# snt-arg/visual_sgraphs

Measured on NVIDIA B200. Metric: orb_extraction_frames_per_s_640x480_1000f, higher is better.
Workload: dtype u8

## Files before the change

visual_sgraphs_b200/csrc/resize_tma.cu:

```cuda
#include <cuda.h>
#include <cuda_runtime.h>

#include <algorithm>
#include <cstdint>
#include <cstdlib>
#include <vector>

#include "tma_util.cuh"
#include "vsg_internal.cuh"

namespace vsg {

constexpr int kRtW = 128, kRtH = 32;
constexpr int kRtBoxW = 192, kRtBoxH = 48;
constexpr int kRtWarps = 8;
constexpr int kRtThreads = 32 * (kRtWarps + 1);
constexpr int kRtHPitch = kRtW + 4;
constexpr int kRtWin = kRtBoxW * kRtBoxH;
constexpr int kRtSmem = 2 * kRtWin + kRtBoxH * kRtHPitch * 4 + 128;

struct RtTileInfo {
    int x0, y0, frame, xs, ys, nrows, ylast, pad;
    short4 yt[kRtH];
};

__global__ void __launch_bounds__(kRtThreads, 4) resize_tma_kernel(const __grid_constant__ CUtensorMap src_map, uint8_t *__restrict__ dst,
                                                                   int dst_pitch, int64_t dst_stride, int dw, int dh, int tiles_x,
                                                                   int tiles_y, int total_tiles, int per_cta,
                                                                   const short4 *__restrict__ xtab, const short4 *__restrict__ ytab) {
    extern __shared__ uint8_t rt_smem_raw[];
    uint8_t *win = reinterpret_cast<uint8_t *>(((uintptr_t)rt_smem_raw + 127) & ~(uintptr_t)127);
    uint32_t *hp = reinterpret_cast<uint32_t *>(win + 2 * kRtWin);
    __shared__ uint64_t full[2], empty[2];
    __shared__ RtTileInfo info[2];
    const int tid = threadIdx.x, lane = tid & 31, warp = tid >> 5;
    const int t_begin = blockIdx.x * per_cta, t_end = min(t_begin + per_cta, total_tiles);
    if (tid == 0) {
        for (int i = 0; i < 2; ++i) { mbar_init(&full[i], 1); mbar_init(&empty[i], kRtWarps); }
        mbar_init_fence();
    }
    __syncthreads();
    const int tiles_per_frame = tiles_x * tiles_y;

    if (warp == kRtWarps) {
        for (int t = t_begin, it = 0; t < t_end; ++t, ++it) {
            const int st = it & 1;
            const int frame = t / tiles_per_frame, rem = t - frame * tiles_per_frame;
            const int tx = rem / tiles_y, ty = rem - tx * tiles_y;
            const int x0 = tx * kRtW, y0 = ty * kRtH, ylast = min(y0 + kRtH, dh) - 1;
            const short4 ytl = __ldg(&ytab[min(y0 + lane, dh - 1)]);
            const int xs = __ldg(&xtab[x0]).x & ~15;
            const int ys = __shfl_sync(0xffffffffu, (int)ytl.x, 0);
            const int nrows = __shfl_sync(0xffffffffu, (int)ytl.y, ylast - y0) - ys + 1;
            mbar_wait(&empty[st], ((it >> 1) & 1) ^ 1);
            info[st].yt[lane] = ytl;
            if (lane == 0) {
                info[st].x0 = x0; info[st].y0 = y0; info[st].frame = frame; info[st].xs = xs; info[st].ys = ys;
                info[st].nrows = nrows; info[st].ylast = ylast;
            }
            __syncwarp();
            if (lane == 0) {
                mbar_expect_tx(&full[st], kRtWin);
                tma_load_3d(win + st * kRtWin, &src_map, xs, ys, frame, &full[st]);
            }
        }
        return;
    }

    int cur_x0 = -1;
    bool col_ok = false;
    uint32_t sel[4], coef[4];
    bool hi[4];
    int base = 0;
    for (int t = t_begin, it = 0; t < t_end; ++t, ++it) {
        const int st = it & 1;
        mbar_wait(&full[st], (it >> 1) & 1);
        const int x0 = info[st].x0, y0 = info[st].y0, frame = info[st].frame, xs = info[st].xs, ys = info[st].ys, nrows = info[st].nrows,
                  ylast = info[st].ylast;
        const int x4 = x0 + 4 * lane;
        if (x0 != cur_x0) {
            cur_x0 = x0;
            col_ok = x4 < dw;
            short4 xt[4];
#pragma unroll
            for (int k = 0; k < 4; ++k) xt[k] = col_ok ? __ldg(&xtab[x4 + k]) : make_short4(0, 0, 0, 0);
            base = xt[0].x & ~3;
#pragma unroll
            for (int k = 0; k < 4; ++k) {
                const int o0 = xt[k].x - base, o1 = xt[k].y - base;
                hi[k] = o1 >= 8;
                const int f = hi[k] ? 4 : 0;
                sel[k] = (uint32_t)(o0 - f) | ((uint32_t)(o1 - f) << 4);
                coef[k] = (uint32_t)(uint16_t)xt[k].z | ((uint32_t)(uint16_t)xt[k].w << 16);
            }
        }
        const uint8_t *wcol = win + st * kRtWin + (col_ok ? base - xs : 0);
        for (int r = warp; r < nrows; r += kRtWarps) {
            const uint32_t *p = reinterpret_cast<const uint32_t *>(wcol + r * kRtBoxW);
            const uint32_t w0 = p[0], w1 = p[1], w2 = p[2];
            uint4 g;
            uint32_t *gp = &g.x;
#pragma unroll
            for (int k = 0; k < 4; ++k) {
                const uint32_t bytes = hi[k] ? __byte_perm(w1, w2, sel[k]) : __byte_perm(w0, w1, sel[k]);
                gp[k] = __dp2a_lo(coef[k], bytes, 0u) >> 4;
            }
            *reinterpret_cast<uint4 *>(hp + r * kRtHPitch + 4 * lane) = g;
        }
        short4 yt[kRtH / kRtWarps];
#pragma unroll
        for (int i = 0; i < kRtH / kRtWarps; ++i) yt[i] = info[st].yt[warp + kRtWarps * i];
        __syncwarp();
        if (lane == 0) mbar_arrive(&empty[st]);
        asm volatile("bar.sync 1, %0;" ::"n"(32 * kRtWarps) : "memory");
        uint8_t *d = dst + (int64_t)frame * dst_stride + x4;
#pragma unroll
        for (int i = 0; i < kRtH / kRtWarps; ++i) {
            const int y = y0 + warp + kRtWarps * i;
            if (y > ylast || !col_ok) continue;
            const uint4 ga = *reinterpret_cast<const uint4 *>(hp + (yt[i].x - ys) * kRtHPitch + 4 * lane);
            const uint4 gb = *reinterpret_cast<const uint4 *>(hp + (yt[i].y - ys) * kRtHPitch + 4 * lane);
            const uint32_t b0 = (uint32_t)yt[i].z << 16, b1 = (uint32_t)yt[i].w << 16;
            const uint32_t v0 = (__umulhi(b0, ga.x) + __umulhi(b1, gb.x) + 2u) >> 2, v1 = (__umulhi(b0, ga.y) + __umulhi(b1, gb.y) + 2u) >> 2;
            const uint32_t v2 = (__umulhi(b0, ga.z) + __umulhi(b1, gb.z) + 2u) >> 2, v3 = (__umulhi(b0, ga.w) + __umulhi(b1, gb.w) + 2u) >> 2;
            *reinterpret_cast<uint32_t *>(d + (int64_t)y * dst_pitch) = v0 | (v1 << 8) | (v2 << 16) | (v3 << 24);
        }
        asm volatile("bar.sync 1, %0;" ::"n"(32 * kRtWarps) : "memory");
    }
}

static int resize_tma_min_frames() {
    const char *e = getenv("VSG_RESIZE_TMA");
    const int v = e ? atoi(e) : 16;
    return v <= 0 ? INT32_MAX : v;
}

bool launch_resize_level_tma(const FrameGeom &g, int level, const uint8_t *src_base, int src_pitch, int64_t src_stride, uint8_t *pyr,
                             int nframes, cudaStream_t s) {
    if (nframes < resize_tma_min_frames()) return false;
    const LevelGeom &L = g.lv[level], &P = g.lv[level - 1];
    if (!L.resize_tma_ok || ((uintptr_t)src_base & 15) || (src_pitch & 15) || (src_stride & 15) || src_pitch < kRtBoxW) return false;
    EncodeTiledFn fn = encode_tiled_fn();
    if (!fn) return false;
    CUtensorMap map;
    const cuuint64_t dims[3] = {(cuuint64_t)src_pitch, (cuuint64_t)P.h, (cuuint64_t)nframes};
    const cuuint64_t strides[2] = {(cuuint64_t)src_pitch, (cuuint64_t)src_stride};
    const cuuint32_t box[3] = {kRtBoxW, kRtBoxH, 1};
    const cuuint32_t estr[3] = {1, 1, 1};
    if (fn(&map, CU_TENSOR_MAP_DATA_TYPE_UINT8, 3, (void *)src_base, dims, strides, box, estr, CU_TENSOR_MAP_INTERLEAVE_NONE,
           CU_TENSOR_MAP_SWIZZLE_NONE, CU_TENSOR_MAP_L2_PROMOTION_L2_128B, CU_TENSOR_MAP_FLOAT_OOB_FILL_NONE) != CUDA_SUCCESS)
        return false;
    if (cudaFuncSetAttribute(resize_tma_kernel, cudaFuncAttributeMaxDynamicSharedMemorySize, kRtSmem) != cudaSuccess) {
        cudaGetLastError();
        return false;
    }
    const int tiles_x = (L.w + kRtW - 1) / kRtW, tiles_y = (L.h + kRtH - 1) / kRtH;
    const int64_t total = (int64_t)tiles_x * tiles_y * nframes;
    if (total > INT32_MAX) return false;
    int dev = 0, sms = 148;
    cudaGetDevice(&dev);
    cudaDeviceGetAttribute(&sms, cudaDevAttrMultiProcessorCount, dev);
    const int ctas = (int)std::min<int64_t>(total, (int64_t)sms * 4);
    const int per_cta = (int)((total + ctas - 1) / ctas);
    resize_tma_kernel<<<(unsigned)((total + per_cta - 1) / per_cta), kRtThreads, kRtSmem, s>>>(
        map, pyr + L.plane_offset, L.pitch, L.plane_stride, L.w, L.h, tiles_x, tiles_y, (int)total, per_cta, L.xtab, L.ytab);
    count_launch();
    return true;
}

bool resize_tma_fits(const std::vector<short4> &xt, const std::vector<short4> &yt, int dw, int dh) {
    for (int x0 = 0; x0 < dw; x0 += kRtW) {
        const int xl = std::min(x0 + kRtW, dw) - 1;
        if ((xt[xl].y & ~3) + 12 - (xt[x0].x & ~15) > kRtBoxW) return false;
    }
    for (int y0 = 0; y0 < dh; y0 += kRtH) {
        const int yl = std::min(y0 + kRtH, dh) - 1;
        if (yt[yl].y - yt[y0].x + 1 > kRtBoxH) return false;
    }
    return true;
}

}
```

visual_sgraphs_b200/csrc/vsg_api.cu:

```cuda
#include <algorithm>
#include <atomic>
#include <cmath>
#include <cstdarg>
#include <cstdio>
#include <cstdlib>
#include <cstring>
#include <vector>

#include "vsg_internal.cuh"

namespace vsg {

static thread_local char g_err[512] = "";
static std::atomic<int64_t> g_launches{0};

void set_error(const char *fmt, ...) {
    va_list ap;
    va_start(ap, fmt);
    vsnprintf(g_err, sizeof(g_err), fmt, ap);
    va_end(ap);
}
bool cuda_ok(cudaError_t e, const char *what) {
    if (e == cudaSuccess) return true;
    set_error("%s: %s", what, cudaGetErrorString(e));
    return false;
}
void count_launch(int n) { g_launches += n; }
static thread_local bool g_pdl_small_batch = true;
constexpr int kPdlMaxFrames = 8;
void pdl_scope(int nframes) { g_pdl_small_batch = nframes <= kPdlMaxFrames; }
bool pdl_enabled() { return g_pdl_small_batch; }

static inline int cv_round(float v) { return (int)lrintf(v); }
static inline int cv_round(double v) { return (int)lrint(v); }
static inline int64_t align_up(int64_t v, int64_t a) { return (v + a - 1) / a * a; }

}

using namespace vsg;

struct vsg_extractor {
    int device = 0;
    int max_batch = 1;
    cudaStream_t stream = nullptr;
    static constexpr int kAuxStreams = 2;
    cudaStream_t aux[kAuxStreams] = {nullptr, nullptr};
    int chunk_frames = 128;
    uint8_t *color_d = nullptr;
    size_t color_bytes = 0;
    uint32_t *rect_xy[2] = {nullptr, nullptr};
    uint16_t *rect_frac[2] = {nullptr, nullptr};
    int rect_w = 0, rect_h = 0;
    cudaEvent_t fork_ev = nullptr;
    vsg_orb_params p{};
    std::vector<float> scale, inv_scale, sigma2, inv_sigma2;
    std::vector<int> quota;

    int cur_w = 0, cur_h = 0;
    FrameGeom g{};
    int max_cw = 0, max_ch = 0, max_nodes = 0;
    int64_t pyr_bytes_per_frame = 0;

    short4 *tabs_d = nullptr;
    PyrTile *pyr_tiles_d = nullptr;
    int pyr_ntiles = 0, pyr_tile_buf = 0;
    size_t pyr_tile_smem = 0;
    uint8_t *pyr = nullptr, *blur = nullptr;
    Cand *cand = nullptr;
    unsigned short *node_of = nullptr;
    int *cand_count = nullptr;
    LevelKp *level_kps = nullptr;
    int *level_kp_count = nullptr;
    int *slot = nullptr;
    uint8_t *out_block_d = nullptr, *out_block_h = nullptr;
    size_t out_block_bytes = 0;
    vsg_keypoint *kps_d = nullptr;
    uint8_t *desc_d = nullptr;
    int *n_d = nullptr, *mono_d = nullptr;
    vsg_keypoint *kps_h = nullptr;
    uint8_t *desc_h = nullptr;
    int *n_h = nullptr, *mono_h = nullptr;

    bool profile = false;
    static constexpr int kEvRing = 32;
    cudaEvent_t ev[kEvRing][VSG_NUM_STAGES + 1] = {};
    bool ev_created = false;
    int ev_head = 0, ev_pending = 0;
    double stage_ms[VSG_NUM_STAGES] = {0, 0, 0, 0, 0};
    int64_t stage_runs = 0;

    void harvest_one() {
        const int slot = (ev_head - ev_pending + 2 * kEvRing) % kEvRing;
        cudaEventSynchronize(ev[slot][VSG_NUM_STAGES]);
        for (int k = 0; k < VSG_NUM_STAGES; ++k) {
            float ms = 0.f;
            cudaEventElapsedTime(&ms, ev[slot][k], ev[slot][k + 1]);
            stage_ms[k] += ms;
        }
        ++stage_runs;
        --ev_pending;
    }

    const uint8_t *lvl0_base = nullptr;
    int lvl0_pitch = 0;
    int64_t lvl0_stride = 0;
    int last_nframes = 0;
    bool results_on_handle = false;

    void free_shape() {
        cudaFree(tabs_d); cudaFree(pyr_tiles_d); cudaFree(pyr); cudaFree(blur); cudaFree(cand); cudaFree(node_of);
        cudaFree(cand_count); cudaFree(level_kps); cudaFree(level_kp_count); cudaFree(slot); cudaFree(out_block_d);
        cudaFree(color_d);
        color_d = nullptr; color_bytes = 0;
        cudaFreeHost(out_block_h);
        out_block_d = out_block_h = nullptr; out_block_bytes = 0;
        tabs_d = nullptr; pyr_tiles_d = nullptr; pyr_ntiles = 0; pyr = blur = nullptr; cand = nullptr; node_of = nullptr;
        cand_count = nullptr; level_kps = nullptr; level_kp_count = nullptr; slot = nullptr; kps_d = nullptr;
        desc_d = nullptr; n_d = mono_d = nullptr; kps_h = nullptr; desc_h = nullptr; n_h = mono_h = nullptr;
        cur_w = cur_h = 0;
    }
};

namespace {

void build_tables(vsg_extractor *ex) {
    const int nl = ex->p.nlevels;
    const double scale_factor = ex->p.scale_factor;
    ex->scale.assign(nl, 1.f);
    ex->sigma2.assign(nl, 1.f);
    for (int i = 1; i < nl; ++i) {
        ex->scale[i] = (float)(ex->scale[i - 1] * scale_factor);
        ex->sigma2[i] = ex->scale[i] * ex->scale[i];
    }
    ex->inv_scale.resize(nl);
    ex->inv_sigma2.resize(nl);
    for (int i = 0; i < nl; ++i) {
        ex->inv_scale[i] = 1.0f / ex->scale[i];
        ex->inv_sigma2[i] = 1.0f / ex->sigma2[i];
    }
    ex->quota.assign(nl, 0);
    const float factor = (float)(1.0f / scale_factor);
    float desired = ex->p.nfeatures * (1 - factor) / (1 - (float)std::pow((double)factor, (double)nl));
    int sum = 0;
    for (int l = 0; l < nl - 1; ++l) {
        ex->quota[l] = cv_round(desired);
        sum += ex->quota[l];
        desired *= factor;
    }
    ex->quota[nl - 1] = std::max(ex->p.nfeatures - sum, 0);
}

void build_resize_tables(int sw, int sh, int dw, int dh, int dw_pad, std::vector<short4> &xt, std::vector<short4> &yt) {
    const double scale_x = 1.0 / ((double)dw / sw), scale_y = 1.0 / ((double)dh / sh);
    xt.resize(dw_pad);
    yt.resize(dh);
    for (int dx = 0; dx < dw_pad; ++dx) {
        const int x = std::min(dx, dw - 1);
        float fx = (float)((x + 0.5) * scale_x - 0.5);
        int sx = (int)std::floor(fx);
        fx -= sx;
        if (sx < 0) { fx = 0; sx = 0; }
        if (sx >= sw - 1) { fx = 0; sx = sw - 1; }
        xt[dx] = make_short4((short)sx, (short)std::min(sx + 1, sw - 1), (short)cv_round((1.f - fx) * 2048.f),
                             (short)cv_round(fx * 2048.f));
    }
    for (int dy = 0; dy < dh; ++dy) {
        float fy = (float)((dy + 0.5) * scale_y - 0.5);
        int sy = (int)std::floor(fy);
        fy -= sy;
        const int sy0 = std::min(std::max(sy, 0), sh - 1), sy1 = std::min(std::max(sy + 1, 0), sh - 1);
        yt[dy] = make_short4((short)sy0, (short)sy1, (short)cv_round((1.f - fy) * 2048.f), (short)cv_round(fy * 2048.f));
    }
}

vsg_status configure_shape(vsg_extractor *ex, int w, int h) {
    if (ex->cur_w == w && ex->cur_h == h) return VSG_OK;
    if (w > kMaxImageDim || h > kMaxImageDim) {
        set_error("image %dx%d too large: at most %d pixels per side", w, h, kMaxImageDim);
        return VSG_ERR_INVALID;
    }
    CK(cudaSetDevice(ex->device));
    int smem_optin = 0;
    size_t octree_static = 0;
    CK(cudaDeviceGetAttribute(&smem_optin, cudaDevAttrMaxSharedMemoryPerBlockOptin, ex->device));
    const vsg_status ost = octree_static_smem_bytes(&octree_static);
    if (ost != VSG_OK) return ost;
    ex->free_shape();
    const int nl = ex->p.nlevels;
    FrameGeom &g = ex->g;
    memset(&g, 0, sizeof(g));
    g.nlevels = nl;
    std::vector<Cell> cells;
    ex->max_cw = ex->max_ch = 7;
    ex->max_nodes = 8;
    int64_t plane_off = 0, cand_off = 0;
    int kp_off = 0;
    std::vector<std::vector<short4>> xts(nl), yts(nl);
    for (int l = 0; l < nl; ++l) {
        LevelGeom &L = g.lv[l];
        L.w = cv_round((float)w * ex->inv_scale[l]);
        L.h = cv_round((float)h * ex->inv_scale[l]);
        const int min_b = kBorderMin, max_bx = L.w - kBorderMin, max_by = L.h - kBorderMin;
        const float width = (float)(max_bx - min_b), height = (float)(max_by - min_b);
        if (width < 35.f || height < 35.f) {
            set_error("image %dx%d too small: level %d is %dx%d (needs >= 67x67 for one 35-px cell)", w, h, l, L.w, L.h);
            return VSG_ERR_INVALID;
        }
        L.pitch = (int)align_up(L.w, 64);
        L.plane_stride = align_up((int64_t)L.pitch * L.h, 256);
        L.plane_offset = plane_off;
        plane_off += L.plane_stride * ex->max_batch;
        L.n_cols = (int)(width / 35.f);
        L.n_rows = (int)(height / 35.f);
        L.w_cell = (int)std::ceil(width / L.n_cols);
        L.h_cell = (int)std::ceil(height / L.n_rows);
        L.cell_begin = (int)cells.size();
        int cand_cap = 0;
        for (int i = 0; i < L.n_rows; ++i) {
            const float ini_y = (float)(min_b + i * L.h_cell);
            float max_y = ini_y + L.h_cell + 6;
            if (ini_y >= max_by - 3) continue;
            if (max_y > max_by) max_y = (float)max_by;
            for (int j = 0; j < L.n_cols; ++j) {
                const float ini_x = (float)(min_b + j * L.w_cell);
                float max_x = ini_x + L.w_cell + 6;
                if (ini_x >= max_bx - 6) continue;
                if (max_x > max_bx) max_x = (float)max_bx;
                Cell c;
                c.level = (short)l;
                c.x0 = (short)ini_x; c.y0 = (short)ini_y;
                c.cw = (short)((int)max_x - (int)ini_x); c.ch = (short)((int)max_y - (int)ini_y);
                c.pad = 0;
                if (c.cw < 7 || c.ch < 7) continue;
                cells.push_back(c);
                ex->max_cw = std::max<int>(ex->max_cw, c.cw);
                ex->max_ch = std::max<int>(ex->max_ch, c.ch);
                cand_cap += ((c.cw - 6 + 1) / 2) * ((c.ch - 6 + 1) / 2);
            }
        }
        L.cell_count = (int)cells.size() - L.cell_begin;
        L.cols_eff = L.rows_eff = 0;
        for (int k = L.cell_begin; k < (int)cells.size(); ++k) {
            const Cell &c = cells[k];
            L.cols_eff = std::max(L.cols_eff, (c.x0 - min_b) / L.w_cell + 1);
            L.rows_eff = std::max(L.rows_eff, (c.y0 - min_b) / L.h_cell + 1);
        }
        if (L.cols_eff * L.rows_eff != L.cell_count) {
            set_error("internal: level %d cell table is not a prefix rectangle", l);
            return VSG_ERR_INVALID;
        }
        L.cols_rcp = (uint32_t)((0x100000000ull + (uint64_t)L.cols_eff - 1) / (uint64_t)std::max(L.cols_eff, 1));
        L.wcell_rcp = L.w_cell > 1 ? (uint32_t)((0x100000000ull + (uint64_t)L.w_cell - 1) / (uint64_t)L.w_cell) : 0xFFFFFFFFu;
        L.hcell_rcp = L.h_cell > 1 ? (uint32_t)((0x100000000ull + (uint64_t)L.h_cell - 1) / (uint64_t)L.h_cell) : 0xFFFFFFFFu;
        L.quota = ex->quota[l];
        L.n_ini = (int)std::round(static_cast<float>(max_bx - min_b) / (max_by - min_b));
        if (L.n_ini < 1) {
            set_error("image %dx%d: aspect ratio below 0.5 is not supported by the reference oct-tree (nIni = 0)", w, h);
            return VSG_ERR_INVALID;
        }
        L.h_x = static_cast<float>(max_bx - min_b) / L.n_ini;
        L.cand_cap = cand_cap + 8;
        L.cand_offset = cand_off;
        cand_off += L.cand_cap;
        L.kp_cap = std::max(L.quota, 4 * L.n_ini) + 4;
        L.kp_offset = kp_off;
        kp_off += L.kp_cap;
        const size_t octree_need = octree_smem_bytes(L.kp_cap + 4) + octree_static;
        if (octree_need > (size_t)smem_optin) {
            set_error("level %d: oct-tree quota %d needs %zu bytes of shared memory per block, the device allows %d", l, L.quota,
                      octree_need, smem_optin);
            return VSG_ERR_INVALID;
        }
        ex->max_nodes = std::max(ex->max_nodes, L.kp_cap + 4);
        L.scale = ex->scale[l];
        L.kp_size = (float)(int)(kPatch * ex->scale[l]);
        L.resize_tma_ok = 0;
        if (l > 0) {
            build_resize_tables(g.lv[l - 1].w, g.lv[l - 1].h, L.w, L.h, (int)align_up(L.w, 4), xts[l], yts[l]);
            L.resize_tma_ok = resize_tma_fits(xts[l], yts[l], L.w, L.h) ? 1 : 0;
        }
    }
    g.ncells = (int)cells.size();
    for (int l = nl; l < kMaxLevels; ++l) g.lv[l].cell_begin = 0x7fffffff;
    g.cand_total = cand_off;
    g.kp_total = kp_off;
    g.out_cap = kp_off;
    ex->pyr_bytes_per_frame = plane_off / ex->max_batch;

    const int B = ex->max_batch;
    size_t ntab = 0;
    for (int l = 1; l < nl; ++l) ntab += xts[l].size() + yts[l].size();
    CK(cudaMalloc(&ex->tabs_d, std::max<size_t>(ntab, 1) * sizeof(short4)));
    size_t toff = 0;
    for (int l = 1; l < nl; ++l) {
        CK(cudaMemcpy(ex->tabs_d + toff, xts[l].data(), xts[l].size() * sizeof(short4), cudaMemcpyHostToDevice));
        g.lv[l].xtab = ex->tabs_d + toff;
        toff += xts[l].size();
        CK(cudaMemcpy(ex->tabs_d + toff, yts[l].data(), yts[l].size() * sizeof(short4), cudaMemcpyHostToDevice));
        g.lv[l].ytab = ex->tabs_d + toff;
        toff += yts[l].size();
    }
    if (nl >= 2) {
        constexpr int ntx = 12, nty = 12;
        std::vector<PyrTile> tiles((size_t)ntx * nty);
        int buf = 0, ntab_max = 0, dim_max = 0;
        for (int ty = 0; ty < nty; ++ty)
            for (int tx = 0; tx < ntx; ++tx) {
                PyrTile &t = tiles[(size_t)ty * ntx + tx];
                int ntab_t = 0;
                for (int l = nl - 1; l >= 0; --l) {
                    const int W = g.lv[l].w, H = g.lv[l].h;
                    PyrTileBox o{(short)(tx * W / ntx), (short)(ty * H / nty), (short)((tx + 1) * W / ntx - 1), (short)((ty + 1) * H / nty - 1)};
                    PyrTileBox r = o;
                    if (l < nl - 1) {
                        const PyrTileBox &u = t.region[l + 1];
                        const short nx0 = xts[l + 1][u.x0].x, nx1 = xts[l + 1][u.x1].y, ny0 = yts[l + 1][u.y0].x, ny1 = yts[l + 1][u.y1].y;
                        if (l == 0) r = PyrTileBox{nx0, ny0, nx1, ny1};
                        else r = PyrTileBox{std::min(o.x0, nx0), std::min(o.y0, ny0), std::max(o.x1, nx1), std::max(o.y1, ny1)};
                    }
                    t.owned[l] = o;
                    t.region[l] = r;
                    t.rcp_w[l] = (uint32_t)((0x100000000ull + (uint64_t)(r.x1 - r.x0)) / (uint64_t)(r.x1 - r.x0 + 1));
                    buf = std::max(buf, (r.x1 - r.x0 + 1) * (r.y1 - r.y0 + 1));
                    if (l > 0) dim_max = std::max(dim_max, std::max(r.x1 - r.x0 + 1, r.y1 - r.y0 + 1));
                    if (l > 0) ntab_t += (r.x1 - r.x0 + 1) + (r.y1 - r.y0 + 1);
                }
                for (int l = nl; l < kMaxLevels; ++l) { t.owned[l] = t.region[l] = PyrTileBox{0, 0, -1, -1}; t.rcp_w[l] = 0; }
                ntab_max = std::max(ntab_max, ntab_t);
            }
        ex->pyr_tile_buf = (int)align_up(buf, 16);
        ex->pyr_tile_smem = 2 * (size_t)ex->pyr_tile_buf + (size_t)ntab_max * sizeof(short4);
        if (ex->pyr_tile_smem <= 160 * 1024 && dim_max <= 256 && buf < 65536 && nl <= kMaxLevels && g.lv[nl - 1].w >= 2 * ntx && g.lv[nl - 1].h >= 2 * nty) {
            CK(cudaMalloc(&ex->pyr_tiles_d, tiles.size() * sizeof(PyrTile)));
            CK(cudaMemcpy(ex->pyr_tiles_d, tiles.data(), tiles.size() * sizeof(PyrTile), cudaMemcpyHostToDevice));
            ex->pyr_ntiles = (int)tiles.size();
        }
    }
    CK(cudaMalloc(&ex->pyr, plane_off + 256));
    CK(cudaMalloc(&ex->blur, plane_off + 256));
    CK(cudaMemset(ex->pyr, 0, plane_off + 256));
    CK(cudaMalloc(&ex->cand, (size_t)g.cand_total * B * sizeof(Cand)));
    CK(cudaMalloc(&ex->node_of, (size_t)g.cand_total * B * sizeof(unsigned short)));
    CK(cudaMalloc(&ex->cand_count, (size_t)B * nl * sizeof(int)));
    CK(cudaMalloc(&ex->level_kps, (size_t)g.kp_total * B * sizeof(LevelKp)));
    CK(cudaMalloc(&ex->level_kp_count, (size_t)B * nl * sizeof(int)));
    CK(cudaMalloc(&ex->slot, (size_t)g.kp_total * B * sizeof(int)));
    {
        auto up = [](size_t v) { return (v + 255) & ~(size_t)255; };
        const size_t off_desc = up((size_t)g.out_cap * B * sizeof(vsg_keypoint));
        const size_t off_n = off_desc + up((size_t)g.out_cap * B * 32);
        const size_t off_mono = off_n + up((size_t)B * sizeof(int));
        ex->out_block_bytes = off_mono + up((size_t)B * sizeof(int));
        CK(cudaMalloc(&ex->out_block_d, ex->out_block_bytes));
        CK(cudaMallocHost(&ex->out_block_h, ex->out_block_bytes));
        ex->kps_d = reinterpret_cast<vsg_keypoint *>(ex->out_block_d);
        ex->desc_d = ex->out_block_d + off_desc;
        ex->n_d = reinterpret_cast<int *>(ex->out_block_d + off_n);
        ex->mono_d = reinterpret_cast<int *>(ex->out_block_d + off_mono);
        ex->kps_h = reinterpret_cast<vsg_keypoint *>(ex->out_block_h);
        ex->desc_h = ex->out_block_h + off_desc;
        ex->n_h = reinterpret_cast<int *>(ex->out_block_h + off_n);
        ex->mono_h = reinterpret_cast<int *>(ex->out_block_h + off_mono);
    }
    ex->cur_w = w;
    ex->cur_h = h;
    return VSG_OK;
}

static int pyr_tile_max_frames() {
    const char *e = getenv("VSG_PYR_TILE");
    return e ? atoi(e) : 4;
}

vsg_status run_pipeline(vsg_extractor *ex, cudaStream_t s, int f0, const uint8_t *lvl0_base, int lvl0_pitch,
                        int64_t lvl0_stride, int nframes, int lap_x0, int lap_x1, vsg_keypoint *kps_dev,
                        uint8_t *desc_dev, int out_cap, int *n_dev, int *mono_dev) {
    FrameGeom g = ex->g;
    for (int l = 0; l < g.nlevels; ++l) {
        g.lv[l].plane_offset += (int64_t)f0 * g.lv[l].plane_stride;
        g.lv[l].cand_offset += (int64_t)f0 * g.cand_total;
    }
    pdl_scope(nframes);
    int *cand_count = ex->cand_count + (size_t)f0 * g.nlevels;
    int *level_kp_count = ex->level_kp_count + (size_t)f0 * g.nlevels;
    LevelKp *level_kps = ex->level_kps + (size_t)f0 * g.kp_total;
    int *slot = ex->slot + (size_t)f0 * g.kp_total;
    CK(cudaMemsetAsync(cand_count, 0, (size_t)nframes * g.nlevels * sizeof(int), s));
    cudaEvent_t *ev = nullptr;
    if (ex->profile && s == ex->stream) {
        if (!ex->ev_created) {
            for (int i = 0; i < vsg_extractor::kEvRing; ++i)
                for (int k = 0; k <= VSG_NUM_STAGES; ++k) CK(cudaEventCreate(&ex->ev[i][k]));
            ex->ev_created = true;
        }
        if (ex->ev_pending == vsg_extractor::kEvRing) ex->harvest_one();
        ev = ex->ev[ex->ev_head];
        ex->ev_head = (ex->ev_head + 1) % vsg_extractor::kEvRing;
        ++ex->ev_pending;
    }
#define STAGE_MARK(k) do { if (ev) CK(cudaEventRecord(ev[k], s)); } while (0)
    STAGE_MARK(0);
    if (ex->pyr_tiles_d && nframes <= pyr_tile_max_frames()) {
        launch_pyramid_tiles(g, ex->pyr_tiles_d, ex->pyr_ntiles, ex->pyr_tile_buf, ex->pyr_tile_smem, lvl0_base, lvl0_pitch, lvl0_stride,
                             ex->pyr, nframes, s);
    } else {
        for (int l = 1; l < g.nlevels; ++l) {
            const LevelGeom &P = g.lv[l - 1];
            if (l == 1) launch_resize_level(g, l, lvl0_base, lvl0_pitch, lvl0_stride, ex->pyr, nframes, s);
            else launch_resize_level(g, l, ex->pyr + P.plane_offset, P.pitch, P.plane_stride, ex->pyr, nframes, s);
        }
    }
    STAGE_MARK(1);
    const BlurTcPlan *blur_tc = plan_blur_tc(g, lvl0_base, lvl0_pitch, lvl0_stride, ex->pyr, ex->blur, nframes);
    const vsg_status fst = launch_fast(g, lvl0_base, lvl0_pitch, lvl0_stride, ex->pyr, blur_tc ? nullptr : ex->blur, ex->cand,
                                       cand_count, ex->p.ini_th_fast, ex->p.min_th_fast, ex->max_cw, ex->max_ch, nframes, s);
    if (fst != VSG_OK) return fst;
    STAGE_MARK(2);
    const vsg_status ost = launch_octree(g, ex->cand, cand_count, ex->node_of, level_kps, level_kp_count, ex->max_nodes, nframes, s);
    if (ost != VSG_OK) return ost;
    STAGE_MARK(3);
    if (blur_tc) launch_blur_tc(blur_tc, ex->blur, s);
    STAGE_MARK(4);
    launch_describe(g, lvl0_base, lvl0_pitch, lvl0_stride, ex->pyr, ex->blur, level_kps, level_kp_count, lap_x0,
                    lap_x1, kps_dev, desc_dev, out_cap, n_dev, mono_dev, slot, nframes, s);
    STAGE_MARK(5);
#undef STAGE_MARK
    CK(cudaGetLastError());
    return VSG_OK;
}

}

namespace vsg {
bool extractor_pyramid(vsg_extractor *ex, PyramidRef *out) {
    if (!ex || ex->cur_w == 0 || ex->last_nframes == 0) return false;
    out->device = ex->device;
    out->nframes = ex->last_nframes;
    out->geom = &ex->g;
    out->lvl0_base = ex->lvl0_base;
    out->lvl0_pitch = ex->lvl0_pitch;
    out->lvl0_stride = ex->lvl0_stride;
    out->pyr = ex->pyr;
    out->scale = ex->scale.data();
    out->inv_scale = ex->inv_scale.data();
    out->stream = ex->stream;
    out->kps_dev = ex->results_on_handle ? ex->kps_d : nullptr;
    out->desc_dev = ex->results_on_handle ? ex->desc_d : nullptr;
    out->n_dev = ex->results_on_handle ? ex->n_d : nullptr;
    out->out_cap = ex->g.out_cap;
    return true;
}
}

extern "C" {

const char *vsg_last_error(void) { return g_err; }

int vsg_device_count(void) {
    int n = 0;
    if (cudaGetDeviceCount(&n) != cudaSuccess) { cudaGetLastError(); return 0; }
    return n;
}

int64_t vsg_launch_count(void) { return g_launches.load(); }

vsg_status vsg_extractor_create(const vsg_orb_params *params, int device, int max_batch, vsg_extractor **out) {
    if (!params || !out || max_batch < 1 || params->nlevels < 1 || params->nlevels > kMaxLevels ||
        params->scale_factor <= 1.0f || params->scale_factor >= 2.0f || params->nfeatures < 0) {
        set_error("vsg_extractor_create: invalid argument");
        return VSG_ERR_INVALID;
    }
    if (vsg_device_count() <= device || device < 0) {
        set_error("vsg_extractor_create: CUDA device %d not available (this library has no CPU fallback)", device);
        return VSG_ERR_CUDA;
    }
    vsg_extractor *ex = new vsg_extractor();
    ex->device = device;
    ex->max_batch = max_batch;
    ex->p = *params;
    build_tables(ex);
    if (!cuda_ok(cudaSetDevice(device), "cudaSetDevice") ||
        !cuda_ok(cudaStreamCreateWithFlags(&ex->stream, cudaStreamNonBlocking), "cudaStreamCreate") ||
        !cuda_ok(cudaStreamCreateWithFlags(&ex->aux[0], cudaStreamNonBlocking), "cudaStreamCreate") ||
        !cuda_ok(cudaStreamCreateWithFlags(&ex->aux[1], cudaStreamNonBlocking), "cudaStreamCreate")) {
        delete ex;
        return VSG_ERR_CUDA;
    }
    if (const char *e = getenv("VSG_CHUNK_FRAMES")) ex->chunk_frames = std::max(1, atoi(e));
    cudaEventCreateWithFlags(&ex->fork_ev, cudaEventDisableTiming);
    *out = ex;
    return VSG_OK;
}

void vsg_extractor_destroy(vsg_extractor *ex) {
    if (!ex) return;
    cudaSetDevice(ex->device);
    if (ex->stream) { cudaStreamSynchronize(ex->stream); cudaStreamDestroy(ex->stream); }
    for (cudaStream_t a : ex->aux)
        if (a) { cudaStreamSynchronize(a); cudaStreamDestroy(a); }
    if (ex->fork_ev) cudaEventDestroy(ex->fork_ev);
    if (ex->ev_created)
        for (int i = 0; i < vsg_extractor::kEvRing; ++i)
            for (int k = 0; k <= VSG_NUM_STAGES; ++k) cudaEventDestroy(ex->ev[i][k]);
    ex->free_shape();
    for (int k = 0; k < 2; ++k) { cudaFree(ex->rect_xy[k]); cudaFree(ex->rect_frac[k]); }
    delete ex;
}

vsg_status vsg_extractor_tables(const vsg_extractor *ex, float *scale, float *inv_scale, float *sigma2,
                                float *inv_sigma2, int32_t *features_per_level) {
    if (!ex) return VSG_ERR_INVALID;
    for (int i = 0; i < ex->p.nlevels; ++i) {
        if (scale) scale[i] = ex->scale[i];
        if (inv_scale) inv_scale[i] = ex->inv_scale[i];
        if (sigma2) sigma2[i] = ex->sigma2[i];
        if (inv_sigma2) inv_sigma2[i] = ex->inv_sigma2[i];
        if (features_per_level) features_per_level[i] = ex->quota[i];
    }
    return VSG_OK;
}

int vsg_extractor_max_keypoints(vsg_extractor *ex, int width, int height) {
    if (!ex) return VSG_ERR_INVALID;
    vsg_status st = configure_shape(ex, width, height);
    if (st != VSG_OK) return st;
    return ex->g.out_cap;
}

static vsg_status extract_batch_host(vsg_extractor *ex, const uint8_t *images, int nframes, int src_w, int src_h, int pitch,
                                     size_t frame_stride, int channels, int r_first, int rect_slots, int lap_x0, int lap_x1,
                                     vsg_keypoint *keypoints_out, uint8_t *descriptors_out, int capacity, int *n_out,
                                     int *mono_index_out) {
    if (!ex) return VSG_ERR_INVALID;
    if (!images || src_w <= 0 || src_h <= 0 || nframes <= 0) return VSG_EMPTY_IMAGE;
    if (nframes > ex->max_batch || pitch < src_w * channels || capacity < 0 || (channels != 1 && channels != 3 && channels != 4)) {
        set_error("vsg_extract_batch: nframes %d > max_batch %d, or bad pitch/capacity/channels", nframes, ex->max_batch);
        return VSG_ERR_INVALID;
    }
    const bool staged = channels != 1 || rect_slots > 0;
    const int width = rect_slots > 0 ? ex->rect_w : src_w, height = rect_slots > 0 ? ex->rect_h : src_h;
    CK(cudaSetDevice(ex->device));
    vsg_status st = configure_shape(ex, width, height);
    if (st != VSG_OK) return st;
    const int cpitch = (src_w * channels + 63) & ~63;
    const size_t cstride = (size_t)cpitch * src_h;
    if (staged && ex->color_bytes < cstride * ex->max_batch) {
        cudaFree(ex->color_d);
        ex->color_d = nullptr; ex->color_bytes = 0;
        CK(cudaMalloc(&ex->color_d, cstride * ex->max_batch));
        ex->color_bytes = cstride * ex->max_batch;
    }
    const FrameGeom &g = ex->g;
    const LevelGeom &L0 = g.lv[0];
    uint8_t *lvl0 = ex->pyr + L0.plane_offset;
    ex->lvl0_base = lvl0; ex->lvl0_pitch = L0.pitch; ex->lvl0_stride = L0.plane_stride; ex->last_nframes = nframes;
    ex->results_on_handle = true;
    auto pinned = [](const void *p) {
        if (!p) return false;
        cudaPointerAttributes a;
        if (cudaPointerGetAttributes(&a, p) != cudaSuccess) { cudaGetLastError(); return false; }
        return a.type == cudaMemoryTypeHost;
    };
    const bool direct = capacity >= g.out_cap && (!keypoints_out || pinned(keypoints_out)) &&
                        (!descriptors_out || pinned(descriptors_out));
    const int min_chunk = std::min(ex->chunk_frames, 64);
    const bool chunked = !ex->profile && nframes >= 2 * min_chunk;
    int chunk = nframes;
    if (chunked) {
        const int nchunks = std::max(2, (nframes + ex->chunk_frames - 1) / ex->chunk_frames);
        chunk = (nframes + nchunks - 1) / nchunks;
    }
    const bool tight = frame_stride == (size_t)pitch * height && (int64_t)L0.pitch * L0.h == L0.plane_stride;
    RectifyMaps maps = {{ex->rect_xy[0], ex->rect_xy[1]}, {ex->rect_frac[0], ex->rect_frac[1]}, rect_slots};
    int nstreams_used = 0;
    if (chunked) {
        CK(cudaEventRecord(ex->fork_ev, ex->stream));
        for (cudaStream_t a : ex->aux) CK(cudaStreamWaitEvent(a, ex->fork_ev, 0));
    }
    for (int f0 = 0, c = 0; f0 < nframes; f0 += chunk, ++c) {
        const int nf = std::min(chunk, nframes - f0);
        cudaStream_t s = (c % 3 == 0) ? ex->stream : ex->aux[c % 3 - 1];
        nstreams_used = std::min(3, c + 1);
// ... 279 lines not shown
```

visual_sgraphs_b200/csrc/vsg_internal.cuh:

```cuda
#pragma once
#include <cuda_runtime.h>
#include <stdint.h>

#include <vector>

#include "../../include/vsg_cuda.h"

namespace vsg {

constexpr int kMaxLevels = 16;
constexpr int kEdge = 19;
constexpr int kBorderMin = 16;
constexpr int kMaxImageDim = 16384;
constexpr int kHalfPatch = 15;
constexpr int kPatch = 31;

struct LevelGeom {
    int w, h;
    int pitch;
    int64_t plane_stride;
    int64_t plane_offset;
    int n_cols, n_rows, w_cell, h_cell;
    int cell_begin, cell_count;
    int cols_eff, rows_eff;
    uint32_t cols_rcp;
    uint32_t wcell_rcp, hcell_rcp;
    int quota;
    int n_ini;
    float h_x;
    int cand_cap;
    int64_t cand_offset;
    int kp_cap;
    int kp_offset;
    float scale;
    float kp_size;
    int resize_tma_ok;
    const short4 *xtab;
    const short4 *ytab;
};

struct FrameGeom {
    int nlevels;
    int ncells;
    int64_t cand_total;
    int kp_total;
    int out_cap;
    LevelGeom lv[kMaxLevels];
};

struct Cell {
    short level;
    short x0, y0;
    short cw, ch;
    short pad;
};

struct __align__(8) Cand {
    unsigned short x, y;
    unsigned short score;
    unsigned short pad;
};

struct __align__(8) LevelKp {
    unsigned short x, y;
    unsigned short score;
    unsigned short pad;
};

}

struct vsg_matcher {
    int device = 0;
    cudaStream_t stream = nullptr;
    void *buf[20] = {};
    size_t cap[20] = {};
    void *hbuf[8] = {};
    size_t hcap[8] = {};
    std::vector<char> scratch[2];
    int sm_count = 148;
};

namespace vsg {

vsg_status matcher_ensure(vsg_matcher *m, int slot, size_t bytes);
vsg_status matcher_ensure_host(vsg_matcher *m, int slot, size_t bytes);
vsg_status launch_knn2_merge_parts(vsg_matcher *m, const int32_t *idx_parts, const int32_t *dist_parts, int nparts, int nq,
                                   int32_t *out_idx, int32_t *out_dist);
bool knn2_tc_supported(int nq, int nt);
vsg_status knn2_tc_device(vsg_matcher *m, const uint8_t *q_dev, int nq, const uint8_t *t_dev, int nt, int offset, int *idx_dev,
                          int *dist_dev);
void launch_window_dists(vsg_matcher *m, const uint8_t *query_dev, int nq, const uint8_t *train_dev,
                         const int *cand_ptr_dev, const int *cand_dev, int *all_dist_dev);

struct PyramidRef {
    int device;
    int nframes;
    const FrameGeom *geom;
    const uint8_t *lvl0_base;
    int lvl0_pitch;
    int64_t lvl0_stride;
    const uint8_t *pyr;
    const float *scale, *inv_scale;
    cudaStream_t stream;
    const vsg_keypoint *kps_dev;
    const uint8_t *desc_dev;
    const int *n_dev;
    int out_cap;
};
bool extractor_pyramid(vsg_extractor *ex, PyramidRef *out);

__device__ __forceinline__ void pdl_launch_dependents() { asm volatile("griddepcontrol.launch_dependents;" ::: "memory"); }
__device__ __forceinline__ void pdl_wait() { asm volatile("griddepcontrol.wait;" ::: "memory"); }
bool pdl_enabled();
void pdl_scope(int nframes);

template <class... KArgs, class... Args>
inline cudaError_t launch_kernel(void (*kernel)(KArgs...), dim3 grid, dim3 block, size_t smem, cudaStream_t s, bool pdl,
                                 Args... args) {
    cudaLaunchConfig_t cfg = {};
    cfg.gridDim = grid;
    cfg.blockDim = block;
    cfg.dynamicSmemBytes = smem;
    cfg.stream = s;
    cudaLaunchAttribute attr[1];
    attr[0].id = cudaLaunchAttributeProgrammaticStreamSerialization;
    attr[0].val.programmaticStreamSerializationAllowed = 1;
    cfg.attrs = attr;
    cfg.numAttrs = (pdl && pdl_enabled()) ? 1 : 0;
    return cudaLaunchKernelEx(&cfg, kernel, KArgs(args)...);
}

void set_error(const char *fmt, ...);
bool cuda_ok(cudaError_t e, const char *what);
#define CK(call)                                          \
    do {                                                  \
        if (!cuda_ok((call), #call)) return VSG_ERR_CUDA; \
    } while (0)
void count_launch(int n = 1);

struct PyrTileBox { short x0, y0, x1, y1; };
struct PyrTile {
    PyrTileBox region[kMaxLevels], owned[kMaxLevels];
    uint32_t rcp_w[kMaxLevels];
};
void launch_pyramid_tiles(const FrameGeom &g, const PyrTile *tiles, int ntiles, int buf_bytes, size_t smem, const uint8_t *lvl0_base,
                          int lvl0_pitch, int64_t lvl0_stride, uint8_t *pyr, int nframes, cudaStream_t s);
bool launch_resize_level_tma(const FrameGeom &g, int level, const uint8_t *src_base, int src_pitch, int64_t src_stride, uint8_t *pyr,
                             int nframes, cudaStream_t s);
bool resize_tma_fits(const std::vector<short4> &xt, const std::vector<short4> &yt, int dw, int dh);
void launch_resize_level(const FrameGeom &g, int level, const uint8_t *src_base, int src_pitch, int64_t src_stride,
                         uint8_t *pyr, int nframes, cudaStream_t s);
void launch_cvt_gray(const uint8_t *src, int src_pitch, int64_t src_stride, int channels, int r_first, uint8_t *dst,
                     int dst_pitch, int64_t dst_stride, int w, int h, int nframes, cudaStream_t s);
struct RectifyMaps {
    const uint32_t *xy[2];
    const uint16_t *frac[2];
    int nslots;
};
void launch_remap(const uint8_t *src, int src_pitch, int64_t src_stride, int sw, int sh, const RectifyMaps &maps, int first_frame,
                  uint8_t *dst, int dst_pitch, int64_t dst_stride, int w, int h, int nframes, cudaStream_t s);
struct BlurTcPlan;
const BlurTcPlan *plan_blur_tc(const FrameGeom &g, const uint8_t *lvl0_base, int lvl0_pitch, int64_t lvl0_stride, const uint8_t *pyr,
                               const uint8_t *blur, int nframes);
void launch_blur_tc(const BlurTcPlan *plan, uint8_t *blur, cudaStream_t s);
void launch_blur(const FrameGeom &g, const uint8_t *lvl0_base, int lvl0_pitch, int64_t lvl0_stride, const uint8_t *pyr,
                 uint8_t *blur, int nframes, cudaStream_t s);
vsg_status launch_fast(const FrameGeom &g, const uint8_t *lvl0_base, int lvl0_pitch, int64_t lvl0_stride, const uint8_t *pyr,
                       uint8_t *blur, Cand *cand, int *cand_count, int ini_th, int min_th, int max_cw, int max_ch, int nframes,
                       cudaStream_t s);
size_t octree_smem_bytes(int max_nodes);
vsg_status octree_static_smem_bytes(size_t *bytes);
vsg_status launch_octree(const FrameGeom &g, const Cand *cand, const int *cand_count, unsigned short *node_of,
                         LevelKp *level_kps, int *level_kp_count, int max_nodes, int nframes, cudaStream_t s);
void launch_describe(const FrameGeom &g, const uint8_t *lvl0_base, int lvl0_pitch, int64_t lvl0_stride,
                     const uint8_t *pyr, const uint8_t *blur, const LevelKp *level_kps, const int *level_kp_count,
                     int lap_x0, int lap_x1, vsg_keypoint *kps_out, uint8_t *desc_out, int out_cap, int *n_out,
                     int *mono_out, int *slot_scratch, int nframes, cudaStream_t s);

}
```

Baseline: 157,600.

## Restructure TMA resize into per-warp column strips with streaming row ring

Replaces the producer-warp, double-buffered 2D tile scheme with a design where each warp owns a vertical column strip of a frame segment. Each warp streams 8-row TMA bands through a private 4-slot mbarrier ring and keeps the previous and current horizontally filtered rows in registers. This drops the shared horizontal-pass buffer, the block-wide barriers, and the redundant horizontal work on halo rows. The cost is a requirement of monotonic, at-most-one-row-step vertical tables, less parallelism per frame, and a sequential per-warp row loop.

```diff
diff --git a/visual_sgraphs_b200/csrc/resize_tma.cu b/visual_sgraphs_b200/csrc/resize_tma.cu
--- a/visual_sgraphs_b200/csrc/resize_tma.cu
+++ b/visual_sgraphs_b200/csrc/resize_tma.cu
@@ -11,121 +11,116 @@
 
 namespace vsg {
 
-constexpr int kRtW = 128, kRtH = 32;
-constexpr int kRtBoxW = 192, kRtBoxH = 48;
-constexpr int kRtWarps = 8;
-constexpr int kRtThreads = 32 * (kRtWarps + 1);
-constexpr int kRtHPitch = kRtW + 4;
-constexpr int kRtWin = kRtBoxW * kRtBoxH;
-constexpr int kRtSmem = 2 * kRtWin + kRtBoxH * kRtHPitch * 4 + 128;
+constexpr int kRsBand = 8;
+constexpr int kRsSlots = 4;
+constexpr int kRsMaxWarps = 16;
+constexpr int kRsMaxBox = 256;
+constexpr int kRsSegRows = 64;
 
-struct RtTileInfo {
-    int x0, y0, frame, xs, ys, nrows, ylast, pad;
-    short4 yt[kRtH];
-};
+static void strip_split(int dw, int *gs, int *ns) {
+    const int groups = (dw + 3) / 4;
+    *ns = (groups + 31) / 32;
+    *gs = (groups + *ns - 1) / *ns;
+}
 
-__global__ void __launch_bounds__(kRtThreads, 4) resize_tma_kernel(const __grid_constant__ CUtensorMap src_map, uint8_t *__restrict__ dst,
-                                                                   int dst_pitch, int64_t dst_stride, int dw, int dh, int tiles_x,
-                                                                   int tiles_y, int total_tiles, int per_cta,
-                                                                   const short4 *__restrict__ xtab, const short4 *__restrict__ ytab) {
-    extern __shared__ uint8_t rt_smem_raw[];
-    uint8_t *win = reinterpret_cast<uint8_t *>(((uintptr_t)rt_smem_raw + 127) & ~(uintptr_t)127);
-    uint32_t *hp = reinterpret_cast<uint32_t *>(win + 2 * kRtWin);
-    __shared__ uint64_t full[2], empty[2];
-    __shared__ RtTileInfo info[2];
-    const int tid = threadIdx.x, lane = tid & 31, warp = tid >> 5;
-    const int t_begin = blockIdx.x * per_cta, t_end = min(t_begin + per_cta, total_tiles);
-    if (tid == 0) {
-        for (int i = 0; i < 2; ++i) { mbar_init(&full[i], 1); mbar_init(&empty[i], kRtWarps); }
+__device__ __forceinline__ void mbar_wait_suspend(uint64_t *bar, uint32_t parity) {
+    asm volatile(
+        "{\n\t.reg .pred p;\n\t"
+        "RS_WAIT:\n\t"
+        "mbarrier.try_wait.parity.shared::cta.b64 p, [%0], %1, %2;\n\t"
+        "@p bra RS_DONE;\n\t"
+        "bra RS_WAIT;\n\t"
+        "RS_DONE:\n\t}" ::"r"(smem_u32(bar)),
+        "r"(parity), "r"(1000000u)
+        : "memory");
+}
+
+__global__ void __launch_bounds__(32 * kRsMaxWarps) resize_tma_kernel(const __grid_constant__ CUtensorMap src_map, uint8_t *__restrict__ dst,
+                                                                      int dst_pitch, int64_t dst_stride, int dw, int dh, int gs, int box,
+                                                                      int seg_h, const short4 *__restrict__ xtab,
+                                                                      const short4 *__restrict__ ytab) {
+    extern __shared__ uint8_t rs_smem_raw[];
+    __shared__ uint64_t full[kRsMaxWarps][kRsSlots];
+    const int lane = threadIdx.x & 31, warp = threadIdx.x >> 5;
+    const int frame = blockIdx.x;
+    const int y0 = blockIdx.y * seg_h, y1 = min(y0 + seg_h, dh);
+    const int x0 = 4 * gs * warp, x4 = x0 + 4 * lane;
+    const int slot_bytes = kRsBand * box;
+    uint8_t *ring = reinterpret_cast<uint8_t *>(((uintptr_t)rs_smem_raw + 127) & ~(uintptr_t)127) + warp * kRsSlots * slot_bytes;
+    uint64_t *bar = full[warp];
+
+    const int ys = __ldg(&ytab[y0]).x, nbands = (__ldg(&ytab[y1 - 1]).y - ys) / kRsBand + 1;
+    const int xs = __ldg(&xtab[x0]).x & ~15;
+    if (lane == 0) {
+        for (int i = 0; i < kRsSlots; ++i) mbar_init(&bar[i], 1);
         mbar_init_fence();
+        for (int b = 0; b < min(kRsSlots, nbands); ++b) {
+            mbar_expect_tx(&bar[b], slot_bytes);
+            tma_load_3d(ring + b * slot_bytes, &src_map, xs, ys + b * kRsBand, frame, &bar[b]);
+        }
     }
-    __syncthreads();
-    const int tiles_per_frame = tiles_x * tiles_y;
-
-    if (warp == kRtWarps) {
-        for (int t = t_begin, it = 0; t < t_end; ++t, ++it) {
-            const int st = it & 1;
-            const int frame = t / tiles_per_frame, rem = t - frame * tiles_per_frame;
-            const int tx = rem / tiles_y, ty = rem - tx * tiles_y;
-            const int x0 = tx * kRtW, y0 = ty * kRtH, ylast = min(y0 + kRtH, dh) - 1;
-            const short4 ytl = __ldg(&ytab[min(y0 + lane, dh - 1)]);
-            const int xs = __ldg(&xtab[x0]).x & ~15;
-            const int ys = __shfl_sync(0xffffffffu, (int)ytl.x, 0);
-            const int nrows = __shfl_sync(0xffffffffu, (int)ytl.y, ylast - y0) - ys + 1;
-            mbar_wait(&empty[st], ((it >> 1) & 1) ^ 1);
-            info[st].yt[lane] = ytl;
-            if (lane == 0) {
-                info[st].x0 = x0; info[st].y0 = y0; info[st].frame = frame; info[st].xs = xs; info[st].ys = ys;
-                info[st].nrows = nrows; info[st].ylast = ylast;
-            }
-            __syncwarp();
-            if (lane == 0) {
-                mbar_expect_tx(&full[st], kRtWin);
-                tma_load_3d(win + st * kRtWin, &src_map, xs, ys, frame, &full[st]);
-            }
-        }
-        return;
-    }
-
-    int cur_x0 = -1;
-    bool col_ok = false;
+    const bool col_ok = lane < gs && x4 < dw;
+    short4 xt[4];
+#pragma unroll
+    for (int k = 0; k < 4; ++k) xt[k] = col_ok ? __ldg(&xtab[x4 + k]) : make_short4(0, 0, 0, 0);
+    const int base = xt[0].x & ~3;
     uint32_t sel[4], coef[4];
     bool hi[4];
-    int base = 0;
-    for (int t = t_begin, it = 0; t < t_end; ++t, ++it) {
-        const int st = it & 1;
-        mbar_wait(&full[st], (it >> 1) & 1);
-        const int x0 = info[st].x0, y0 = info[st].y0, frame = info[st].frame, xs = info[st].xs, ys = info[st].ys, nrows = info[st].nrows,
-                  ylast = info[st].ylast;
-        const int x4 = x0 + 4 * lane;
-        if (x0 != cur_x0) {
-            cur_x0 = x0;
-            col_ok = x4 < dw;
-            short4 xt[4];
 #pragma unroll
-            for (int k = 0; k < 4; ++k) xt[k] = col_ok ? __ldg(&xtab[x4 + k]) : make_short4(0, 0, 0, 0);
-            base = xt[0].x & ~3;
+    for (int k = 0; k < 4; ++k) {
+        const int o0 = xt[k].x - base, o1 = xt[k].y - base;
+        hi[k] = k > 0 && o1 >= 8;
+        const int f = hi[k] ? 4 : 0;
+        sel[k] = (uint32_t)(o0 - f) | ((uint32_t)(o1 - f) << 4);
+        coef[k] = (uint32_t)(uint16_t)xt[k].z | ((uint32_t)(uint16_t)xt[k].w << 16);
+    }
+    const uint32_t ring_s = smem_u32(ring), lane_off = col_ok ? (uint32_t)(base - xs) : 0u;
+    __syncwarp();
+
+    int slot = 0, band = 0, rib = 0, cur = ys - 1;
+    uint32_t phase = 0, raddr = ring_s + lane_off;
+    uint32_t hp[4] = {0u, 0u, 0u, 0u}, hc[4] = {0u, 0u, 0u, 0u};
+    mbar_wait_suspend(&bar[0], 0);
+    uint8_t *d = dst + (int64_t)frame * dst_stride + (int64_t)y0 * dst_pitch + x4;
+    const uint2 *yt2 = reinterpret_cast<const uint2 *>(ytab);
+    uint2 yt = __ldg(&yt2[y0]);
+    for (int y = y0; y < y1; ++y) {
+        const uint2 ytn = __ldg(&yt2[min(y + 1, y1 - 1)]);
+        const int sy1 = (int)(yt.x >> 16);
+#pragma unroll 1
+        while (cur < sy1) {
+            if (rib == kRsBand) {
+                asm volatile("fence.proxy.async.shared::cta;" ::: "memory");
+                __syncwarp();
+                if (lane == 0 && band + kRsSlots < nbands) {
+                    mbar_expect_tx(&bar[slot], slot_bytes);
+                    tma_load_3d(ring + slot * slot_bytes, &src_map, xs, ys + (band + kRsSlots) * kRsBand, frame, &bar[slot]);
+                }
+                ++band;
+                if (++slot == kRsSlots) { slot = 0; phase ^= 1u; }
+                rib = 0;
+                raddr = ring_s + slot * slot_bytes + lane_off;
+                mbar_wait_suspend(&bar[slot], phase);
+            }
+            const uint32_t w0 = lds_u32(raddr), w1 = lds_u32(raddr + 4), w2 = lds_u32(raddr + 8);
 #pragma unroll
             for (int k = 0; k < 4; ++k) {
-                const int o0 = xt[k].x - base, o1 = xt[k].y - base;
-                hi[k] = o1 >= 8;
-                const int f = hi[k] ? 4 : 0;
-                sel[k] = (uint32_t)(o0 - f) | ((uint32_t)(o1 - f) << 4);
-                coef[k] = (uint32_t)(uint16_t)xt[k].z | ((uint32_t)(uint16_t)xt[k].w << 16);
+                hp[k] = hc[k];
+                const uint32_t bytes = hi[k] ? __byte_perm(w1, w2, sel[k]) : __byte_perm(w0, w1, sel[k]);
+                hc[k] = __dp2a_lo(coef[k], bytes, 0u) >> 4;
             }
+            raddr += box;
+            ++rib;
+            ++cur;
         }
-        const uint8_t *wcol = win + st * kRtWin + (col_ok ? base - xs : 0);
-        for (int r = warp; r < nrows; r += kRtWarps) {
-            const uint32_t *p = reinterpret_cast<const uint32_t *>(wcol + r * kRtBoxW);
-            const uint32_t w0 = p[0], w1 = p[1], w2 = p[2];
-            uint4 g;
-            uint32_t *gp = &g.x;
+        const bool same = (yt.x & 0xffffu) == (uint32_t)sy1;
+        const uint32_t b0 = yt.y << 16, b1 = yt.y & 0xffff0000u;
+        uint32_t v[4];
 #pragma unroll
-            for (int k = 0; k < 4; ++k) {
-                const uint32_t bytes = hi[k] ? __byte_perm(w1, w2, sel[k]) : __byte_perm(w0, w1, sel[k]);
-                gp[k] = __dp2a_lo(coef[k], bytes, 0u) >> 4;
-            }
-            *reinterpret_cast<uint4 *>(hp + r * kRtHPitch + 4 * lane) = g;
-        }
-        short4 yt[kRtH / kRtWarps];
-#pragma unroll
-        for (int i = 0; i < kRtH / kRtWarps; ++i) yt[i] = info[st].yt[warp + kRtWarps * i];
-        __syncwarp();
-        if (lane == 0) mbar_arrive(&empty[st]);
-        asm volatile("bar.sync 1, %0;" ::"n"(32 * kRtWarps) : "memory");
-        uint8_t *d = dst + (int64_t)frame * dst_stride + x4;
-#pragma unroll
-        for (int i = 0; i < kRtH / kRtWarps; ++i) {
-            const int y = y0 + warp + kRtWarps * i;
-            if (y > ylast || !col_ok) continue;
-            const uint4 ga = *reinterpret_cast<const uint4 *>(hp + (yt[i].x - ys) * kRtHPitch + 4 * lane);
-            const uint4 gb = *reinterpret_cast<const uint4 *>(hp + (yt[i].y - ys) * kRtHPitch + 4 * lane);
-            const uint32_t b0 = (uint32_t)yt[i].z << 16, b1 = (uint32_t)yt[i].w << 16;
-            const uint32_t v0 = (__umulhi(b0, ga.x) + __umulhi(b1, gb.x) + 2u) >> 2, v1 = (__umulhi(b0, ga.y) + __umulhi(b1, gb.y) + 2u) >> 2;
-            const uint32_t v2 = (__umulhi(b0, ga.z) + __umulhi(b1, gb.z) + 2u) >> 2, v3 = (__umulhi(b0, ga.w) + __umulhi(b1, gb.w) + 2u) >> 2;
-            *reinterpret_cast<uint32_t *>(d + (int64_t)y * dst_pitch) = v0 | (v1 << 8) | (v2 << 16) | (v3 << 24);
-        }
-        asm volatile("bar.sync 1, %0;" ::"n"(32 * kRtWarps) : "memory");
+        for (int k = 0; k < 4; ++k) v[k] = (__umulhi(b0, same ? hc[k] : hp[k]) + __umulhi(b1, hc[k]) + 2u) >> 2;
+        if (col_ok) *reinterpret_cast<uint32_t *>(d) = v[0] | (v[1] << 8) | (v[2] << 16) | (v[3] << 24);
+        d += dst_pitch;
+        yt = ytn;
     }
 }
 
@@ -139,45 +134,57 @@
                              int nframes, cudaStream_t s) {
     if (nframes < resize_tma_min_frames()) return false;
     const LevelGeom &L = g.lv[level], &P = g.lv[level - 1];
-    if (!L.resize_tma_ok || ((uintptr_t)src_base & 15) || (src_pitch & 15) || (src_stride & 15) || src_pitch < kRtBoxW) return false;
+    const int box = L.resize_tma_box;
+    if (!L.resize_tma_ok || ((uintptr_t)src_base & 15) || (src_pitch & 15) || (src_stride & 15) || src_pitch < box) return false;
     EncodeTiledFn fn = encode_tiled_fn();
     if (!fn) return false;
     CUtensorMap map;
     const cuuint64_t dims[3] = {(cuuint64_t)src_pitch, (cuuint64_t)P.h, (cuuint64_t)nframes};
     const cuuint64_t strides[2] = {(cuuint64_t)src_pitch, (cuuint64_t)src_stride};
-    const cuuint32_t box[3] = {kRtBoxW, kRtBoxH, 1};
+    const cuuint32_t boxdim[3] = {(cuuint32_t)box, kRsBand, 1};
     const cuuint32_t estr[3] = {1, 1, 1};
-    if (fn(&map, CU_TENSOR_MAP_DATA_TYPE_UINT8, 3, (void *)src_base, dims, strides, box, estr, CU_TENSOR_MAP_INTERLEAVE_NONE,
+    if (fn(&map, CU_TENSOR_MAP_DATA_TYPE_UINT8, 3, (void *)src_base, dims, strides, boxdim, estr, CU_TENSOR_MAP_INTERLEAVE_NONE,
            CU_TENSOR_MAP_SWIZZLE_NONE, CU_TENSOR_MAP_L2_PROMOTION_L2_128B, CU_TENSOR_MAP_FLOAT_OOB_FILL_NONE) != CUDA_SUCCESS)
         return false;
-    if (cudaFuncSetAttribute(resize_tma_kernel, cudaFuncAttributeMaxDynamicSharedMemorySize, kRtSmem) != cudaSuccess) {
+    int gs, ns;
+    strip_split(L.w, &gs, &ns);
+    const int smem = ns * kRsSlots * kRsBand * box + 128;
+    if (cudaFuncSetAttribute(resize_tma_kernel, cudaFuncAttributeMaxDynamicSharedMemorySize, smem) != cudaSuccess) {
         cudaGetLastError();
         return false;
     }
-    const int tiles_x = (L.w + kRtW - 1) / kRtW, tiles_y = (L.h + kRtH - 1) / kRtH;
-    const int64_t total = (int64_t)tiles_x * tiles_y * nframes;
-    if (total > INT32_MAX) return false;
     int dev = 0, sms = 148;
     cudaGetDevice(&dev);
     cudaDeviceGetAttribute(&sms, cudaDevAttrMultiProcessorCount, dev);
-    const int ctas = (int)std::min<int64_t>(total, (int64_t)sms * 4);
-    const int per_cta = (int)((total + ctas - 1) / ctas);
-    resize_tma_kernel<<<(unsigned)((total + per_cta - 1) / per_cta), kRtThreads, kRtSmem, s>>>(
-        map, pyr + L.plane_offset, L.pitch, L.plane_stride, L.w, L.h, tiles_x, tiles_y, (int)total, per_cta, L.xtab, L.ytab);
+    int seg_h = kRsSegRows;
+    while (seg_h > 16 && (int64_t)nframes * ns * ((L.h + seg_h - 1) / seg_h) < (int64_t)sms * 32) seg_h /= 2;
+    const int nseg = (L.h + seg_h - 1) / seg_h;
+    if (nseg > 65535) return false;
+    resize_tma_kernel<<<dim3((unsigned)nframes, (unsigned)nseg), 32 * ns, smem, s>>>(map, pyr + L.plane_offset, L.pitch, L.plane_stride, L.w,
+                                                                                     L.h, gs, box, seg_h, L.xtab, L.ytab);
     count_launch();
     return true;
 }
 
-bool resize_tma_fits(const std::vector<short4> &xt, const std::vector<short4> &yt, int dw, int dh) {
-    for (int x0 = 0; x0 < dw; x0 += kRtW) {
-        const int xl = std::min(x0 + kRtW, dw) - 1;
-        if ((xt[xl].y & ~3) + 12 - (xt[x0].x & ~15) > kRtBoxW) return false;
+int resize_tma_box(const std::vector<short4> &xt, const std::vector<short4> &yt, int dw, int dh) {
+    int gs, ns;
+    strip_split(dw, &gs, &ns);
+    if (ns > kRsMaxWarps) return 0;
+    const int groups = (dw + 3) / 4;
+    int box = 16;
+    for (int w = 0; w < ns; ++w) {
+        const int g0 = w * gs, gl = std::min(g0 + gs, groups) - 1;
+        if (gl < g0) continue;
+        box = std::max(box, (xt[4 * gl].x & ~3) + 12 - (xt[4 * g0].x & ~15));
     }
-    for (int y0 = 0; y0 < dh; y0 += kRtH) {
-        const int yl = std::min(y0 + kRtH, dh) - 1;
-        if (yt[yl].y - yt[y0].x + 1 > kRtBoxH) return false;
+    box = (box + 15) & ~15;
+    if (box > kRsMaxBox) return 0;
+    for (int y = 0; y < dh; ++y) {
+        const int d = yt[y].y - yt[y].x;
+        if (d < 0 || d > 1) return 0;
+        if (y > 0 && (yt[y].x < yt[y - 1].x || yt[y].y < yt[y - 1].y)) return 0;
     }
-    return true;
+    return box;
 }
 
 }
diff --git a/visual_sgraphs_b200/csrc/vsg_api.cu b/visual_sgraphs_b200/csrc/vsg_api.cu
--- a/visual_sgraphs_b200/csrc/vsg_api.cu
+++ b/visual_sgraphs_b200/csrc/vsg_api.cu
@@ -275,9 +275,11 @@
         L.scale = ex->scale[l];
         L.kp_size = (float)(int)(kPatch * ex->scale[l]);
         L.resize_tma_ok = 0;
+        L.resize_tma_box = 0;
         if (l > 0) {
             build_resize_tables(g.lv[l - 1].w, g.lv[l - 1].h, L.w, L.h, (int)align_up(L.w, 4), xts[l], yts[l]);
-            L.resize_tma_ok = resize_tma_fits(xts[l], yts[l], L.w, L.h) ? 1 : 0;
+            L.resize_tma_box = resize_tma_box(xts[l], yts[l], L.w, L.h);
+            L.resize_tma_ok = L.resize_tma_box > 0 ? 1 : 0;
         }
     }
     g.ncells = (int)cells.size();
diff --git a/visual_sgraphs_b200/csrc/vsg_internal.cuh b/visual_sgraphs_b200/csrc/vsg_internal.cuh
--- a/visual_sgraphs_b200/csrc/vsg_internal.cuh
+++ b/visual_sgraphs_b200/csrc/vsg_internal.cuh
@@ -35,6 +35,7 @@
     float scale;
     float kp_size;
     int resize_tma_ok;
+    int resize_tma_box;
     const short4 *xtab;
     const short4 *ytab;
 };
@@ -147,7 +148,7 @@
                           int lvl0_pitch, int64_t lvl0_stride, uint8_t *pyr, int nframes, cudaStream_t s);
 bool launch_resize_level_tma(const FrameGeom &g, int level, const uint8_t *src_base, int src_pitch, int64_t src_stride, uint8_t *pyr,
                              int nframes, cudaStream_t s);
-bool resize_tma_fits(const std::vector<short4> &xt, const std::vector<short4> &yt, int dw, int dh);
+int resize_tma_box(const std::vector<short4> &xt, const std::vector<short4> &yt, int dw, int dh);
 void launch_resize_level(const FrameGeom &g, int level, const uint8_t *src_base, int src_pitch, int64_t src_stride,
                          uint8_t *pyr, int nframes, cudaStream_t s);
 void launch_cvt_gray(const uint8_t *src, int src_pitch, int64_t src_stride, int channels, int r_first, uint8_t *dst,
```

Result: faster. 161,400, median of 6 (+2.4%).
